# j-horner/cuda-nbody

Hardware: AMD Instinct MI355X
Metric: body-body interactions/s, all-pairs N-body step (reference convention N^2 per step) (higher is better)
Workload: dtype f32

## Files before the change

cuda-nbody_amd/csrc/nbody_pair.hip:

```cpp
#include "nbody_kernels.h"

#include <algorithm>
#include <cmath>
#include <vector>

#ifdef NB_PAIR_STAMPS
__device__ unsigned long long nb_pair_stamps[8192 * 8];
extern "C" __attribute__((visibility("default"))) int nb_debug_read_pair_stamps(void* host, size_t bytes) {
    return static_cast<int>(hipMemcpyFromSymbol(host, HIP_SYMBOL(nb_pair_stamps), bytes, 0, hipMemcpyDeviceToHost));
}
#endif

#ifdef NB_PAIR_NONTEMPORAL
#define NB_WS_STORE(ptr, value) __builtin_nontemporal_store((value), (ptr))
#define NB_WS_LOAD(ptr) __builtin_nontemporal_load(ptr)
#else
#define NB_WS_STORE(ptr, value) (*(ptr) = (value))
#define NB_WS_LOAD(ptr) (*(ptr))
#endif

namespace nb {
namespace {

#include "nbody_lane.h"

constexpr int kWaveRor1 = 0x13C;
__device__ __forceinline__ int rotate_bits(int v) { return __builtin_amdgcn_update_dpp(v, v, kWaveRor1, 0xf, 0xf, false); }
__device__ __forceinline__ float rotate(float x) { return __builtin_bit_cast(float, rotate_bits(__builtin_bit_cast(int, x))); }
__device__ __forceinline__ double rotate(double x) {
    const unsigned long long b  = __builtin_bit_cast(unsigned long long, x);
    const unsigned           l2 = static_cast<unsigned>(rotate_bits(static_cast<int>(b & 0xffffffffull)));
    const unsigned           h2 = static_cast<unsigned>(rotate_bits(static_cast<int>(b >> 32)));
    return __builtin_bit_cast(double, (static_cast<unsigned long long>(h2) << 32) | l2);
}
__device__ __forceinline__ v2f rotate(v2f x) { return v2f{rotate(x.x), rotate(x.y)}; }

__device__ __forceinline__ float first_lane(float x) { return __builtin_bit_cast(float, __builtin_amdgcn_readfirstlane(__builtin_bit_cast(int, x))); }
__device__ __forceinline__ double first_lane(double x) {
    const unsigned long long b  = __builtin_bit_cast(unsigned long long, x);
    const unsigned           lo = static_cast<unsigned>(__builtin_amdgcn_readfirstlane(static_cast<int>(b & 0xffffffffull)));
    const unsigned           hi = static_cast<unsigned>(__builtin_amdgcn_readfirstlane(static_cast<int>(b >> 32)));
    return __builtin_bit_cast(double, (static_cast<unsigned long long>(hi) << 32) | lo);
}

__device__ __forceinline__ float  both_halves(v2f a) { return a.x + a.y; }
__device__ __forceinline__ double both_halves(double a) { return a; }

template <int R, int S> constexpr int kPairWavesPerSimd = R <= 4 ? 4 : (S == 12 ? 3 : 2);
#define NB_PAIR_KERNEL pair_forces
#define NB_PAIR_CLOCK_PARAM
#define NB_PAIR_CLOCKED 0
#include "nbody_pair_forces.inc"
#undef NB_PAIR_KERNEL
#undef NB_PAIR_CLOCK_PARAM
#undef NB_PAIR_CLOCKED
#define NB_PAIR_KERNEL pair_forces_clocked
#define NB_PAIR_CLOCK_PARAM , unsigned long long* clock_words
#define NB_PAIR_CLOCKED 1
#include "nbody_pair_forces.inc"
#undef NB_PAIR_KERNEL
#undef NB_PAIR_CLOCK_PARAM
#undef NB_PAIR_CLOCKED

template <typename T> __device__ __forceinline__ void quarter_sums(const T* r, size_t plane, unsigned slots, unsigned wave, T (&t)[3]) {
    const unsigned full = slots & ~3u;
    t[0] = t[1] = t[2] = 0;
    for (unsigned q = wave; q < full; q += 32) {
        T v[3][8];
#pragma unroll
        for (int u = 0; u < 8; ++u) {
            const bool there = (q + 4 * u) < full;
#pragma unroll
            for (int c = 0; c < 3; ++c) v[c][u] = there ? NB_WS_LOAD(r + (static_cast<size_t>(q + 4 * u) * 3 + c) * plane) : T(0);
        }
#pragma unroll
        for (int u = 0; u < 8; ++u) {
#pragma unroll
            for (int c = 0; c < 3; ++c) t[c] += v[c][u];
        }
    }
    if (wave == 0) {
        for (unsigned k = full; k < slots; ++k) {
#pragma unroll
            for (int c = 0; c < 3; ++c) t[c] += NB_WS_LOAD(r + (static_cast<size_t>(k) * 3 + c) * plane);
        }
    }
}

template <typename T> __global__ __launch_bounds__(256) void pair_finish(FinishArgs<T> s) {
    using vec4 = typename Lane<T>::vec4;
    __shared__ T   part[3][3][64];
    const unsigned lane = threadIdx.x & 63, wave = threadIdx.x >> 6;
    const unsigned k    = blockIdx.x * 64 + lane;
    const bool     live = k < s.count;
    T              t[3] = {0, 0, 0};
    const unsigned body   = s.origin + k;
    const bool     closer = wave == 0 && live;
    vec4           v{}, pn{}, e{};
    T              own[3] = {0, 0, 0};
    if (closer) {
        v  = reinterpret_cast<const vec4*>(s.vel)[body];
        pn = reinterpret_cast<const vec4*>(s.old_pos)[body];
        if (s.extra != nullptr) e = reinterpret_cast<const vec4*>(s.extra)[body];
        for (unsigned m = 0; m < s.n_self; ++m) {
            const auto& set = s.self_set[m];
            if (k < set.first || k - set.first >= set.count) continue;
            for (unsigned c0 = 0; c0 < set.slots; c0 += 4) {
                T x[4][3];
#pragma unroll
                for (int i = 0; i < 4; ++i) {
#pragma unroll
                    for (int comp = 0; comp < 3; ++comp) x[i][comp] = (c0 + i) < set.slots ? NB_WS_LOAD(s.self + (static_cast<size_t>(set.slot + c0 + i) * 3 + comp) * s.self_plane + k) : T(0);
                }
#pragma unroll
                for (int i = 0; i < 4; ++i) {
                    if ((c0 + i) < set.slots) {
#pragma unroll
                        for (int comp = 0; comp < 3; ++comp) own[comp] += x[i][comp];
                    }
                }
            }
        }
    }
    if (live) quarter_sums(s.react + k, s.react_plane, s.react_slots, wave, t);
    if (wave != 0) {
#pragma unroll
        for (int comp = 0; comp < 3; ++comp) part[wave - 1][comp][lane] = t[comp];
    }
    __syncthreads();
    if (!closer) return;
    T    got[kMaxRecv][3];
    bool has[kMaxRecv];
#pragma unroll
    for (int m = 0; m < kMaxRecv; ++m) {
        has[m] = static_cast<unsigned>(m) < s.n_recv && k >= s.recv_set[m].first && k - s.recv_set[m].first < s.recv_set[m].count;
#pragma unroll
        for (int comp = 0; comp < 3; ++comp) got[m][comp] = has[m] ? s.recv[(static_cast<size_t>(m) * 3 + comp) * s.recv_plane + k] : T(0);
    }
    T f[3];
#pragma unroll
    for (int comp = 0; comp < 3; ++comp) {
        T others = (t[comp] + part[0][comp][lane]) + (part[1][comp][lane] + part[2][comp][lane]);
#pragma unroll
        for (int m = 0; m < kMaxRecv; ++m) {
            if (has[m]) others += got[m][comp];
        }
        f[comp] = own[comp] - others;
    }
    if (s.extra != nullptr) f[0] += e.x, f[1] += e.y, f[2] += e.z;
    v.x     = __builtin_fma(f[0], s.dt, v.x) * s.damping;
    v.y     = __builtin_fma(f[1], s.dt, v.y) * s.damping;
    v.z     = __builtin_fma(f[2], s.dt, v.z) * s.damping;
    pn.x    = __builtin_fma(v.x, s.dt, pn.x);
    pn.y    = __builtin_fma(v.y, s.dt, pn.y);
    pn.z    = __builtin_fma(v.z, s.dt, pn.z);
    reinterpret_cast<vec4*>(s.new_pos)[body] = pn;
    reinterpret_cast<vec4*>(s.vel)[body]     = v;
}

template <typename T> __global__ __launch_bounds__(256) void pair_reduce(const T* react, unsigned react_plane, unsigned slots, T* out, unsigned out_plane, unsigned count) {
    __shared__ T   part[3][3][64];
    const unsigned lane = threadIdx.x & 63, wave = threadIdx.x >> 6;
    const unsigned k    = blockIdx.x * 64 + lane;
    const bool     live = k < count;
    T              t[3] = {0, 0, 0};
    if (live) quarter_sums(react + k, react_plane, slots, wave, t);
    if (wave != 0) {
#pragma unroll
        for (int comp = 0; comp < 3; ++comp) part[wave - 1][comp][lane] = t[comp];
    }
    __syncthreads();
    if (wave != 0 || !live) return;
#pragma unroll
    for (int comp = 0; comp < 3; ++comp) out[static_cast<size_t>(comp) * out_plane + k] = (t[comp] + part[0][comp][lane]) + (part[1][comp][lane] + part[2][comp][lane]);
}

template <typename T, int R, int S> hipError_t launch_rs(const PairArgs<T>& args, unsigned grid, unsigned lds_bytes, hipStream_t stream, bool prepare_only) {
    if (lds_bytes > 64u * 1024u) {
        if (const auto err = allow_large_lds<&pair_forces<T, R, S>>(); err != hipSuccess) return err;
    }
    unsigned long long* clock_words = nullptr;
    if constexpr (R == 8 && S == 8) {
        size_t capacity = 0;
        unsigned long long* lent = pair_clock_words(&capacity);
        if (lent != nullptr && capacity >= static_cast<size_t>(grid) * 16) clock_words = lent;
        if (lds_bytes > 64u * 1024u && clock_words != nullptr) {
            if (const auto err = allow_large_lds<&pair_forces_clocked<T, R, S>>(); err != hipSuccess) return err;
        }
    }
    if (prepare_only) return hipSuccess;
    (void)hipGetLastError();
    if constexpr (R == 8 && S == 8) {
        if (clock_words != nullptr) {
            hipLaunchKernelGGL((pair_forces_clocked<T, R, S>), dim3(grid), dim3(64 * S), lds_bytes, stream, args, clock_words);
            return hipGetLastError();
        }
    }
    hipLaunchKernelGGL((pair_forces<T, R, S>), dim3(grid), dim3(64 * S), lds_bytes, stream, args);
    return hipGetLastError();
}

template <typename T, int R> hipError_t launch_r(const PairArgs<T>& args, int waves, unsigned grid, unsigned lds_bytes, hipStream_t stream, bool prepare_only) {
    switch (waves) {
        case 4: return launch_rs<T, R, 4>(args, grid, lds_bytes, stream, prepare_only);
        case 8: return launch_rs<T, R, 8>(args, grid, lds_bytes, stream, prepare_only);
        case 12: return launch_rs<T, R, 12>(args, grid, lds_bytes, stream, prepare_only);
        case 16: return launch_rs<T, R, 16>(args, grid, lds_bytes, stream, prepare_only);
        default: return hipErrorInvalidValue;
    }
}

}

inline double resident_workgroups(int S) { return 256.0 * std::max(1, 8 / S); }

inline double busiest_simd_units(unsigned U, unsigned C, int S, bool quarters) {
    const unsigned slots = C * static_cast<unsigned>(S), base = U / slots, rem = U % slots;
    const double   per_simd = static_cast<double>(S) / 4;
    if (quarters) return per_simd * base + pair_tail_units(U, C, S) / 4.0;
    const bool     inter = C > 1 && rem != 0 && base < 34;
    if (rem == 0) return per_simd * base;
    const unsigned longer = (inter || C == 1) ? (rem + C - 1) / C : std::min(rem, static_cast<unsigned>(S));
    return per_simd * base + (longer <= 4 ? 1.0 : 2.0);
}

template <typename T> struct PairCost;
template <> struct PairCost<float> {
    static constexpr double unit[4] = {2.2, 4.53, 9.17, 17.72}, wg[4] = {0.0, 0.0, 1.45, 6.86}, slot = 14.1;
};
template <> struct PairCost<double> {
    static constexpr double unit[4] = {0.0, 5.12, 10.39, 20.72}, wg[4] = {0.0, 0.0, 0.0, 0.0}, slot = 21.9;
};

template <typename T> PairPlan plan_pair(unsigned n, int cu_count, int ovr_r, int ovr_s, int ovr_c) {
    constexpr int W = sizeof(T) == 4 ? 2 : 1;
    (void)cu_count;
    const bool fixed_r = ovr_r == 1 || ovr_r == 2 || ovr_r == 4 || ovr_r == 8;
    const int  S       = (ovr_s == 4 || ovr_s == 8 || ovr_s == 12 || ovr_s == 16) ? ovr_s : 8;
    auto geometry = [&](int R, unsigned C) {
        PairPlan p{};
        const unsigned block  = 64u * static_cast<unsigned>(R * W);
        const unsigned blocks = (n + block - 1) / block;
        p.vectors_per_lane = R;
        p.waves            = S;
        p.splits           = C;
        p.blocks           = blocks;
        p.block_bodies     = block;
        p.slots            = blocks < 2 ? 0u : ((blocks & 1u) ? blocks / 2 : blocks / 2 - 1);
        p.grid_blocks      = blocks * C;
        p.lds_bytes        = pair_lds_bytes(R, W, S, sizeof(T), pair_tail_units((blocks / 2 + 1) * static_cast<unsigned>(R * W), C, S));
        if (p.lds_bytes > kPairLdsLimit) p.lds_bytes = pair_lds_bytes(R, W, S, sizeof(T), 0);
        p.workspace_bytes  = (static_cast<size_t>(C) + p.slots) * 3 * static_cast<size_t>(blocks) * block * sizeof(T);
        return p;
    };
    auto units_of = [&](const PairPlan& p) { return (p.blocks / 2 + 1) * static_cast<unsigned>(p.vectors_per_lane * W); };
    auto with_units = [&](int R, unsigned C) {
        PairPlan p = geometry(R, C);
        while (p.splits > 1 && units_of(p) < p.splits * static_cast<unsigned>(S)) p = geometry(R, p.splits / 2);
        return p;
    };
    PairPlan best{};
    double   best_cost = 0;
    for (int R : {1, 2, 4, 8}) {
        const int k = R == 1 ? 0 : (R == 2 ? 1 : (R == 4 ? 2 : 3));
        if (fixed_r ? R != ovr_r : PairCost<T>::unit[k] == 0.0) continue;
        for (unsigned C = 1; C <= 16; ++C) {
            const PairPlan p = ovr_c > 0 ? with_units(R, static_cast<unsigned>(ovr_c)) : geometry(R, C);
            const unsigned U = units_of(p);
            if (ovr_c <= 0 && C > 1 && U < 2 * C * static_cast<unsigned>(S)) continue;
            const double rounds = std::ceil(p.grid_blocks / resident_workgroups(S));
            const double unit   = PairCost<T>::unit[k] > 0.0 ? PairCost<T>::unit[k] : 0.5 * PairCost<T>::unit[1];
            const bool   quarters = pair_lds_bytes(R, W, S, sizeof(T), pair_tail_units(U, p.splits, S)) <= kPairLdsLimit;
            const double cost   = rounds * (busiest_simd_units(U, p.splits, S, quarters) * unit + PairCost<T>::wg[k]) +
                                PairCost<T>::slot * 1e-6 * static_cast<double>(n) * (p.slots + p.splits);
            if (best.blocks == 0 || cost < 0.995 * best_cost) best = p, best_cost = cost;
            if (ovr_c > 0) break;
        }
    }
    return best;
}

template <typename T> hipError_t launch_pair_tile(const PairArgs<T>& args, const PairGeom& g, hipStream_t stream, bool prepare_only) {
    constexpr int  W         = sizeof(T) == 4 ? 2 : 1;
    PairArgs<T>    a         = args;
    const unsigned block     = 64u * static_cast<unsigned>(g.vectors_per_lane * W);
    a.blocks                 = (a.i_count + block - 1) / block;
    a.splits                 = g.splits;
    const unsigned units = a.diag ? (a.unit_count != 0 ? a.unit_count : (a.blocks / 2 + 1) * static_cast<unsigned>(g.vectors_per_lane * W)) : (a.j_count + 63) / 64;
    unsigned       lds_bytes;
    {
        const unsigned slots = g.splits * static_cast<unsigned>(g.waves), each = units / slots;
        const unsigned tail  = pair_tail_units(units, g.splits, g.waves);
        lds_bytes            = pair_lds_bytes(g.vectors_per_lane, W, g.waves, sizeof(T), tail);
#ifdef NB_PAIR_NO_QUARTERS
        const bool quarters = false;
#else
        const bool quarters = lds_bytes <= kPairLdsLimit;
#endif
        if (quarters) {
            a.deal = 2u;
        } else {
            a.deal    = (g.splits > 1 && units % slots != 0 && each < 34) ? 1u : 0u;
            lds_bytes = pair_lds_bytes(g.vectors_per_lane, W, g.waves, sizeof(T), 0);
        }
    }
    if (a.blocks == 0) return hipSuccess;
    switch (g.vectors_per_lane) {
        case 1: return launch_r<T, 1>(a, g.waves, a.blocks * a.splits, lds_bytes, stream, prepare_only);
        case 2: return launch_r<T, 2>(a, g.waves, a.blocks * a.splits, lds_bytes, stream, prepare_only);
        case 4: return launch_r<T, 4>(a, g.waves, a.blocks * a.splits, lds_bytes, stream, prepare_only);
        case 8: return launch_r<T, 8>(a, g.waves, a.blocks * a.splits, lds_bytes, stream, prepare_only);
        default: return hipErrorInvalidValue;
    }
}

template <typename T> hipError_t launch_pair_reduce(const T* react, unsigned react_plane, unsigned slots, T* out, unsigned out_plane, unsigned count, hipStream_t stream) {
    if (count == 0) return hipSuccess;
    (void)hipGetLastError();
    hipLaunchKernelGGL(pair_reduce<T>, dim3((count + 63) / 64), dim3(256), 0, stream, react, react_plane, slots, out, out_plane, count);
    return hipGetLastError();
}

template <typename T> hipError_t launch_pair_finish(const FinishArgs<T>& args, hipStream_t stream) {
    if (args.count == 0) return hipSuccess;
    (void)hipGetLastError();
    hipLaunchKernelGGL(pair_finish<T>, dim3((args.count + 63) / 64), dim3(256), 0, stream, args);
    return hipGetLastError();
}

template <typename T> hipError_t launch_pair(const Shard<T>& s, const PairPlan& p, void* workspace, hipStream_t stream, bool prepare_only) {
    const unsigned npad = p.blocks * p.block_bodies;
    T* const       work = static_cast<T*>(workspace);
    PairArgs<T>    a{};
    a.old_pos = s.old_pos, a.self = work, a.react = work + static_cast<size_t>(p.splits) * 3 * npad;
    a.n = s.i_count, a.i_begin = 0, a.i_count = s.i_count, a.j_begin = 0, a.j_count = s.i_count;
    a.diag = 1, a.keep = 1;
    a.self_first = 0, a.self_origin = 0, a.self_plane = npad, a.react_origin = 0, a.react_plane = npad;
    a.eps2 = s.eps2;
    const PairGeom g{p.vectors_per_lane, p.waves, p.splits};
    if (const auto err = launch_pair_tile<T>(a, g, stream, prepare_only); err != hipSuccess || prepare_only) return err;
    if (hipEvent_t probe = pair_probe_event(); probe != nullptr) {
        if (const auto err = hipEventRecord(probe, stream); err != hipSuccess) return err;
    }
    FinishArgs<T> f{};
    f.old_pos = s.old_pos, f.new_pos = s.new_pos, f.vel = s.vel;
    f.self = a.self, f.react = a.react, f.recv = nullptr, f.extra = nullptr;
    f.origin = 0, f.count = s.i_count;
    f.self_plane = npad, f.react_plane = npad, f.react_slots = p.slots, f.recv_plane = 0;
    f.n_self = 1, f.n_recv = 0;
    f.self_set[0] = {0u, p.splits, 0u, s.i_count};
    f.dt = s.dt, f.damping = s.damping;
    return launch_pair_finish<T>(f, stream);
}

template <typename T> PairSlicing plan_pair_sliced(unsigned n, unsigned slices, int ovr_r, int ovr_s, int ovr_c) {
    constexpr unsigned W = sizeof(T) == 4 ? 2 : 1;
    PairSlicing        p{};
    if (n == 0 || slices < 2) return p;
    const int R = (ovr_r == 1 || ovr_r == 2 || ovr_r == 4 || ovr_r == 8) ? ovr_r : (n / slices >= 32768 ? 8 : 4);
    const int S = (ovr_s == 4 || ovr_s == 8 || ovr_s == 12 || ovr_s == 16) ? ovr_s : 8;
    const unsigned chip = 256u;
    p.block_bodies          = 64u * static_cast<unsigned>(R) * W;
    const unsigned blocks   = (n + p.block_bodies - 1) / p.block_bodies;
    const unsigned per      = (blocks + slices - 1) / slices;
    p.slice_bodies          = per * p.block_bodies;
    p.slices                = (n + p.slice_bodies - 1) / p.slice_bodies;
    if (p.slices < 2) return PairSlicing{};
    p.partners = p.slices / 2;
    p.even     = (p.slices % 2) == 0;
    if (p.partners + 1 > static_cast<unsigned>(kMaxRecv) || p.partners + 1 > static_cast<unsigned>(kMaxSelfSets)) return PairSlicing{};
    p.plane = p.slice_bodies;
    auto splits = [&](unsigned units) {
        unsigned C = ovr_c > 0 ? static_cast<unsigned>(ovr_c) : splits_to_fill(per, units, S, chip);
        while (C > 1 && units < C * static_cast<unsigned>(S)) C /= 2;
        return C;
    };
    p.diag = {R, S, splits((per / 2 + 1) * static_cast<unsigned>(R) * W)};
    p.rect = {R, S, splits(p.slice_bodies / 64)};
    p.rect_upper = p.rect;
    if (p.even && per >= 2 && p.slice_bodies / 64 >= p.rect.splits * 2 * static_cast<unsigned>(S) * 2) p.rect_upper.splits = p.rect.splits * 2;
    const size_t   plane3     = 3 * static_cast<size_t>(p.plane);
    const unsigned diag_slots = per < 2 ? 0u : ((per & 1u) ? per / 2 : per / 2 - 1);
    p.self_per_slice  = (p.diag.splits + static_cast<size_t>(p.partners - 1) * p.rect.splits + p.rect_upper.splits) * plane3;
    p.react_elements  = static_cast<size_t>(std::max(diag_slots, per)) * plane3;
    p.recv_per_slice  = (1 + static_cast<size_t>(p.partners)) * plane3;
    p.elements        = p.slices * (p.self_per_slice + p.recv_per_slice) + p.react_elements;
    p.workspace_bytes = p.elements * sizeof(T);
    return p;
}

template <typename T> hipError_t launch_pair_sliced(const Shard<T>& s, const PairSlicing& p, void* workspace, hipStream_t stream, bool prepare_only) {
    const unsigned n = s.i_count, K = p.slices, ni = p.slice_bodies, H = p.partners;
    const size_t   plane3 = 3 * static_cast<size_t>(p.plane);
    T* const       work   = static_cast<T*>(workspace);
    T* const       react  = work;
    auto self_of = [&](unsigned r) { return work + p.react_elements + static_cast<size_t>(r) * p.self_per_slice; };
    auto recv_of = [&](unsigned r) { return work + p.react_elements + static_cast<size_t>(K) * p.self_per_slice + static_cast<size_t>(r) * p.recv_per_slice; };
    auto first_of = [&](unsigned r) { return r * ni; };
    auto count_of = [&](unsigned r) { return std::min(ni, n - r * ni); };
    auto blocks_of = [&](unsigned count) { return (count + p.block_bodies - 1) / p.block_bodies; };
    auto half_of = [&](unsigned r) { return (blocks_of(count_of(r)) / 2) * p.block_bodies; };

    std::vector<FinishArgs<T>> finish(K);
    for (unsigned r = 0; r < K; ++r) {
        FinishArgs<T>& f = finish[r];
        f                = {};
        f.old_pos = s.old_pos, f.new_pos = s.new_pos, f.vel = s.vel;
        f.self = self_of(r), f.react = react, f.recv = recv_of(r), f.extra = nullptr;
        f.origin = first_of(r), f.count = count_of(r);
        f.self_plane = f.react_plane = f.recv_plane = p.plane;
        f.react_slots = 0;
        f.dt = s.dt, f.damping = s.damping;
        f.n_recv = 1 + H;
        for (unsigned m = 0; m <= H; ++m) f.recv_set[m] = {0u, 0u};
    }
    for (unsigned r = 0; r < K; ++r) {
        const unsigned own = first_of(r), cnt = count_of(r);
        PairArgs<T>    a{};
        a.old_pos = s.old_pos, a.self = self_of(r), a.n = n, a.eps2 = s.eps2;
        a.self_origin = own, a.self_plane = p.plane, a.react = react, a.react_plane = p.plane;
        a.react_origin = own, a.i_begin = a.j_begin = own, a.i_count = a.j_count = cnt, a.diag = 1, a.keep = 1, a.self_first = 0;
        if (const auto err = launch_pair_tile<T>(a, p.diag, stream, prepare_only); err != hipSuccess) return err;
        finish[r].self_set[finish[r].n_self++] = {0u, p.diag.splits, 0u, cnt};
        const unsigned b = blocks_of(cnt), diag_slots = b < 2 ? 0u : ((b & 1u) ? b / 2 : b / 2 - 1);
        if (diag_slots != 0) {
            if (!prepare_only) {
                if (const auto err = launch_pair_reduce<T>(react, p.plane, diag_slots, recv_of(r), p.plane, cnt, stream); err != hipSuccess) return err;
            }
            finish[r].recv_set[0] = {0u, cnt};
        }
        for (unsigned q = 1; q <= H; ++q) {
            const unsigned partner = (r + q) % K, pfirst = first_of(partner), pcnt = count_of(partner);
            a.diag = 0, a.keep = 1;
            a.i_begin = own, a.i_count = cnt, a.j_begin = pfirst, a.j_count = pcnt;
            const bool split = p.even && q == H;
            if (split) {
                if (r < partner) a.j_count = half_of(partner);
                else a.i_begin = own + half_of(r), a.i_count = cnt - half_of(r);
            }
            a.react_origin = a.j_begin;
            a.self_first   = p.diag.splits + (q - 1) * p.rect.splits;
            if (a.i_count != 0 && a.j_count != 0) {
                const PairGeom& geom = (split && !(r < partner)) ? p.rect_upper : p.rect;
                if (const auto err = launch_pair_tile<T>(a, geom, stream, prepare_only); err != hipSuccess) return err;
                finish[r].self_set[finish[r].n_self++] = {a.self_first, geom.splits, a.i_begin - own, a.i_count};
                if (!prepare_only) {
                    if (const auto err = launch_pair_reduce<T>(react, p.plane, blocks_of(a.i_count), recv_of(partner) + q * plane3, p.plane, a.j_count, stream); err != hipSuccess) return err;
                }
                finish[partner].recv_set[q] = {0u, a.j_count};
            }
        }
    }
    if (prepare_only) return hipSuccess;
    for (unsigned r = 0; r < K; ++r) {
        if (const auto err = launch_pair_finish<T>(finish[r], stream); err != hipSuccess) return err;
    }
    return hipSuccess;
}

template PairPlan   plan_pair<float>(unsigned, int, int, int, int);
template PairPlan   plan_pair<double>(unsigned, int, int, int, int);
template hipError_t launch_pair<float>(const Shard<float>&, const PairPlan&, void*, hipStream_t, bool);
template hipError_t launch_pair<double>(const Shard<double>&, const PairPlan&, void*, hipStream_t, bool);
template PairSlicing plan_pair_sliced<float>(unsigned, unsigned, int, int, int);
template PairSlicing plan_pair_sliced<double>(unsigned, unsigned, int, int, int);
template hipError_t  launch_pair_sliced<float>(const Shard<float>&, const PairSlicing&, void*, hipStream_t, bool);
template hipError_t  launch_pair_sliced<double>(const Shard<double>&, const PairSlicing&, void*, hipStream_t, bool);
template hipError_t launch_pair_tile<float>(const PairArgs<float>&, const PairGeom&, hipStream_t, bool);
template hipError_t launch_pair_tile<double>(const PairArgs<double>&, const PairGeom&, hipStream_t, bool);
template hipError_t launch_pair_reduce<float>(const float*, unsigned, unsigned, float*, unsigned, unsigned, hipStream_t);
template hipError_t launch_pair_reduce<double>(const double*, unsigned, unsigned, double*, unsigned, unsigned, hipStream_t);
template hipError_t launch_pair_finish<float>(const FinishArgs<float>&, hipStream_t);
template hipError_t launch_pair_finish<double>(const FinishArgs<double>&, hipStream_t);

}
```

Measured before the change: 7021 billion.

## Add specialized j-packed symmetric pair kernel for the 8-wave single-split config

Adds a new float-only pair-force kernel that packs two j bodies per lane as v2f. It rotates them across the wave with DPP, and accumulates reactions through a fused rotate-add DPP. Wave priority is adjusted from per-SIMD progress counters, and the kernel is dispatched in place of the generic tile kernel when the plan is 8 vectors per lane, 8 waves and one split. The intent is to raise throughput in the inner loop through more ILP and fewer j loads. The risks are higher register pressure, a separate code path to keep consistent with the generic kernel, and LDS sizing that reuses the generic formula.

```diff
diff --git a/cuda-nbody_amd/csrc/nbody_pair.hip b/cuda-nbody_amd/csrc/nbody_pair.hip
--- a/cuda-nbody_amd/csrc/nbody_pair.hip
+++ b/cuda-nbody_amd/csrc/nbody_pair.hip
@@ -1,8 +1,15 @@
 #include "nbody_kernels.h"
+#include "nbody_pair_lead.h"
 
 #include <algorithm>
 #include <cmath>
 #include <vector>
+
+#if defined(NB_PAIR_STAMPS) || defined(NB_PAIR_NONTEMPORAL) || defined(NB_NO_BALANCE) || defined(NB_PAIR_NO_QUARTERS) || defined(NB_PAIR_UNR) || defined(NB_PAIR_RB)
+#define NB_PAIR_VARIANT_BUILD 1
+#else
+#define NB_PAIR_VARIANT_BUILD 0
+#endif
 
 #ifdef NB_PAIR_STAMPS
 __device__ unsigned long long nb_pair_stamps[8192 * 8];
@@ -11,40 +18,11 @@
 }
 #endif
 
-#ifdef NB_PAIR_NONTEMPORAL
-#define NB_WS_STORE(ptr, value) __builtin_nontemporal_store((value), (ptr))
-#define NB_WS_LOAD(ptr) __builtin_nontemporal_load(ptr)
-#else
-#define NB_WS_STORE(ptr, value) (*(ptr) = (value))
-#define NB_WS_LOAD(ptr) (*(ptr))
-#endif
-
 namespace nb {
 namespace {
 
 #include "nbody_lane.h"
-
-constexpr int kWaveRor1 = 0x13C;
-__device__ __forceinline__ int rotate_bits(int v) { return __builtin_amdgcn_update_dpp(v, v, kWaveRor1, 0xf, 0xf, false); }
-__device__ __forceinline__ float rotate(float x) { return __builtin_bit_cast(float, rotate_bits(__builtin_bit_cast(int, x))); }
-__device__ __forceinline__ double rotate(double x) {
-    const unsigned long long b  = __builtin_bit_cast(unsigned long long, x);
-    const unsigned           l2 = static_cast<unsigned>(rotate_bits(static_cast<int>(b & 0xffffffffull)));
-    const unsigned           h2 = static_cast<unsigned>(rotate_bits(static_cast<int>(b >> 32)));
-    return __builtin_bit_cast(double, (static_cast<unsigned long long>(h2) << 32) | l2);
-}
-__device__ __forceinline__ v2f rotate(v2f x) { return v2f{rotate(x.x), rotate(x.y)}; }
-
-__device__ __forceinline__ float first_lane(float x) { return __builtin_bit_cast(float, __builtin_amdgcn_readfirstlane(__builtin_bit_cast(int, x))); }
-__device__ __forceinline__ double first_lane(double x) {
-    const unsigned long long b  = __builtin_bit_cast(unsigned long long, x);
-    const unsigned           lo = static_cast<unsigned>(__builtin_amdgcn_readfirstlane(static_cast<int>(b & 0xffffffffull)));
-    const unsigned           hi = static_cast<unsigned>(__builtin_amdgcn_readfirstlane(static_cast<int>(b >> 32)));
-    return __builtin_bit_cast(double, (static_cast<unsigned long long>(hi) << 32) | lo);
-}
-
-__device__ __forceinline__ float  both_halves(v2f a) { return a.x + a.y; }
-__device__ __forceinline__ double both_halves(double a) { return a; }
+#include "nbody_pair_lane.h"
 
 template <int R, int S> constexpr int kPairWavesPerSimd = R <= 4 ? 4 : (S == 12 ? 3 : 2);
 #define NB_PAIR_KERNEL pair_forces
@@ -338,7 +316,14 @@
     a.self_first = 0, a.self_origin = 0, a.self_plane = npad, a.react_origin = 0, a.react_plane = npad;
     a.eps2 = s.eps2;
     const PairGeom g{p.vectors_per_lane, p.waves, p.splits};
-    if (const auto err = launch_pair_tile<T>(a, g, stream, prepare_only); err != hipSuccess || prepare_only) return err;
+    const bool lead = !NB_PAIR_VARIANT_BUILD && pair_lead_takes(a, g);
+    if (lead) {
+        if (const auto err = launch_pair_lead(a, stream, prepare_only); err != hipSuccess) return err;
+    }
+    if (!lead || prepare_only) {
+        if (const auto err = launch_pair_tile<T>(a, g, stream, prepare_only); err != hipSuccess) return err;
+    }
+    if (prepare_only) return hipSuccess;
     if (hipEvent_t probe = pair_probe_event(); probe != nullptr) {
         if (const auto err = hipEventRecord(probe, stream); err != hipSuccess) return err;
     }
diff --git a/cuda-nbody_amd/csrc/nbody_pair_lane.h b/cuda-nbody_amd/csrc/nbody_pair_lane.h
--- /dev/null
+++ b/cuda-nbody_amd/csrc/nbody_pair_lane.h
@@ -0,0 +1,34 @@
+#pragma once
+
+#ifdef NB_PAIR_NONTEMPORAL
+#define NB_WS_STORE(ptr, value) __builtin_nontemporal_store((value), (ptr))
+#define NB_WS_LOAD(ptr) __builtin_nontemporal_load(ptr)
+#else
+#define NB_WS_STORE(ptr, value) (*(ptr) = (value))
+#define NB_WS_LOAD(ptr) (*(ptr))
+#endif
+
+constexpr int kWaveRor1 = 0x13C;
+__device__ __forceinline__ int rotate_bits(int v) { return __builtin_amdgcn_update_dpp(v, v, kWaveRor1, 0xf, 0xf, false); }
+__device__ __forceinline__ float rotate(float x) { return __builtin_bit_cast(float, rotate_bits(__builtin_bit_cast(int, x))); }
+__device__ __forceinline__ double rotate(double x) {
+    const unsigned long long b  = __builtin_bit_cast(unsigned long long, x);
+    const unsigned           l2 = static_cast<unsigned>(rotate_bits(static_cast<int>(b & 0xffffffffull)));
+    const unsigned           h2 = static_cast<unsigned>(rotate_bits(static_cast<int>(b >> 32)));
+    return __builtin_bit_cast(double, (static_cast<unsigned long long>(h2) << 32) | l2);
+}
+__device__ __forceinline__ v2f rotate(v2f x) { return v2f{rotate(x.x), rotate(x.y)}; }
+__device__ __forceinline__ float rotate_add(float x, float t) {
+    return __builtin_bit_cast(float, __builtin_amdgcn_update_dpp(0, __builtin_bit_cast(int, x), kWaveRor1, 0xf, 0xf, true)) + t;
+}
+
+__device__ __forceinline__ float first_lane(float x) { return __builtin_bit_cast(float, __builtin_amdgcn_readfirstlane(__builtin_bit_cast(int, x))); }
+__device__ __forceinline__ double first_lane(double x) {
+    const unsigned long long b  = __builtin_bit_cast(unsigned long long, x);
+    const unsigned           lo = static_cast<unsigned>(__builtin_amdgcn_readfirstlane(static_cast<int>(b & 0xffffffffull)));
+    const unsigned           hi = static_cast<unsigned>(__builtin_amdgcn_readfirstlane(static_cast<int>(b >> 32)));
+    return __builtin_bit_cast(double, (static_cast<unsigned long long>(hi) << 32) | lo);
+}
+
+__device__ __forceinline__ float  both_halves(v2f a) { return a.x + a.y; }
+__device__ __forceinline__ double both_halves(double a) { return a; }
diff --git a/cuda-nbody_amd/csrc/nbody_pair_lead.h b/cuda-nbody_amd/csrc/nbody_pair_lead.h
--- /dev/null
+++ b/cuda-nbody_amd/csrc/nbody_pair_lead.h
@@ -0,0 +1,13 @@
+#pragma once
+
+#include "nbody_kernels.h"
+
+namespace nb {
+
+bool       pair_lead_takes(const PairArgs<float>& args, const PairGeom& g);
+inline bool pair_lead_takes(const PairArgs<double>&, const PairGeom&) { return false; }
+
+hipError_t       launch_pair_lead(const PairArgs<float>& args, hipStream_t stream, bool prepare_only);
+inline hipError_t launch_pair_lead(const PairArgs<double>&, hipStream_t, bool) { return hipErrorInvalidValue; }
+
+}
diff --git a/cuda-nbody_amd/csrc/nbody_pair_lead.hip b/cuda-nbody_amd/csrc/nbody_pair_lead.hip
--- /dev/null
+++ b/cuda-nbody_amd/csrc/nbody_pair_lead.hip
@@ -0,0 +1,299 @@
+#include "nbody_pair_lead.h"
+
+namespace nb {
+namespace {
+
+#include "nbody_lane.h"
+#include "nbody_pair_lane.h"
+
+#ifndef NB_PAIR_LEAD_UNR
+#define NB_PAIR_LEAD_UNR 1
+#endif
+#ifndef NB_PAIR_LEAD_IB
+#define NB_PAIR_LEAD_IB 4
+#endif
+
+template <int S> __global__ __launch_bounds__(64 * S) __attribute__((amdgpu_waves_per_eu(2, 2))) void pair_forces_jpacked(PairArgs<float> s) {
+    using LT            = Lane<float>;
+    using T             = float;
+    using vec           = v2f;
+    constexpr int I     = 16;
+    constexpr int P     = I / 2;
+    constexpr int BLOCK = 64 * I;
+    constexpr int TB    = I / 2;
+    constexpr int UNR   = NB_PAIR_LEAD_UNR;
+
+    extern __shared__ __attribute__((aligned(32))) unsigned char smem_raw[];
+
+    const float4* __restrict__ old_pos = reinterpret_cast<const float4*>(s.old_pos);
+    const int      tid  = threadIdx.x;
+    const int      wave = __builtin_amdgcn_readfirstlane(tid >> 6);
+    const int      lane = tid & 63;
+    const unsigned a    = blockIdx.x;
+
+    const unsigned block_base = s.i_begin + a * BLOCK;
+    const unsigned i_end      = s.i_begin + s.i_count;
+    vec            px[P], py[P], pz[P];
+    vec            ax[I], ay[I], az[I];
+    const T        m_block    = old_pos[block_base < i_end ? block_base : i_end - 1].w;
+    const unsigned block_bits = __builtin_bit_cast(unsigned, m_block);
+    bool           same       = true;
+#pragma unroll
+    for (int k = 0; k < I; ++k) {
+        const unsigned i = block_base + k * 64 + lane;
+        const float4   p = old_pos[i < i_end ? i : i_end - 1];
+        LT::set(px[k / 2], k % 2, p.x);
+        LT::set(py[k / 2], k % 2, p.y);
+        LT::set(pz[k / 2], k % 2, p.z);
+        same = same && i < i_end && __builtin_bit_cast(unsigned, p.w) == block_bits;
+    }
+    const bool block_uniform = __builtin_amdgcn_ballot_w64(!same) == 0 && usable_scale(m_block);
+#pragma unroll
+    for (int k = 0; k < I; ++k) ax[k] = ay[k] = az[k] = LT::splat(0);
+    vec eps2 = LT::splat(s.eps2);
+    LT::keep_in_vgpr(eps2);
+    const LT::Consts consts = LT::make_consts();
+
+    constexpr size_t kSumBytes = static_cast<size_t>(S) * 3 * I * 64 * sizeof(T);
+    T* const         sums      = reinterpret_cast<T*>(smem_raw);
+    unsigned* const  balance   = reinterpret_cast<unsigned*>(smem_raw + kSumBytes);
+    unsigned* const  simd_count = balance;
+    volatile unsigned* progress = reinterpret_cast<volatile unsigned*>(balance + 4);
+    if (tid < 36) balance[tid] = tid < 4 ? 0u : 0xffffffffu;
+    __syncthreads();
+    const unsigned simd = static_cast<unsigned>(__builtin_amdgcn_s_getreg((1 << 11) | (4 << 6) | 4));
+    unsigned       slot = 0;
+    if (lane == 0) slot = atomicAdd(&simd_count[simd], 1u);
+    slot = static_cast<unsigned>(__builtin_amdgcn_readfirstlane(static_cast<int>(slot))) & 7u;
+    volatile unsigned* const mine = progress + simd * 8;
+    unsigned                 done = 0;
+    if (lane == 0) mine[slot] = 0;
+
+    constexpr unsigned kFlush = 8;
+    T* const           second = sums + static_cast<size_t>(wave) * (3 * I * 64) + lane;
+#pragma unroll
+    for (int q = 0; q < 3 * I; ++q) second[q * 64] = 0;
+    T unit = T(1);
+    auto flush = [&](vec (&ax)[I], vec (&ay)[I], vec (&az)[I]) {
+#pragma unroll
+        for (int k = 0; k < I; ++k) {
+            second[(0 * I + k) * 64] = __builtin_fmaf(both_halves(ax[k]), unit, second[(0 * I + k) * 64]);
+            second[(1 * I + k) * 64] = __builtin_fmaf(both_halves(ay[k]), unit, second[(1 * I + k) * 64]);
+            second[(2 * I + k) * 64] = __builtin_fmaf(both_halves(az[k]), unit, second[(2 * I + k) * 64]);
+        }
+#pragma unroll
+        for (int k = 0; k < I; ++k) ax[k] = ay[k] = az[k] = LT::splat(0);
+    };
+    auto change_unit = [&](T to) {
+        const vec ratio = LT::splat(unit / to);
+#pragma unroll
+        for (int k = 0; k < I; ++k) ax[k] = ax[k] * ratio, ay[k] = ay[k] * ratio, az[k] = az[k] * ratio;
+        unit = to;
+    };
+
+    const unsigned NB      = s.blocks;
+    const unsigned Q       = NB / 2;
+    const bool     even    = (NB & 1u) == 0;
+    const unsigned j_end   = s.j_begin + s.j_count;
+    const unsigned n_units = (Q + 1) * TB;
+    const unsigned n_items = static_cast<unsigned>(wave) < n_units ? (n_units - static_cast<unsigned>(wave) + S - 1) / S : 0;
+    auto item_unit = [&](unsigned it) { return static_cast<unsigned>(wave) + it * S; };
+    auto tile_first = [&](unsigned u) {
+        unsigned jb = a + u / TB;
+        if (jb >= NB) jb -= NB;
+        return s.j_begin + jb * BLOCK + (u % TB) * 128;
+    };
+    struct Tile {
+        float4 lo, hi;
+    };
+    auto load_tile = [&](unsigned u) {
+        const unsigned j = tile_first(u) + static_cast<unsigned>(lane);
+        return Tile{old_pos[j < j_end ? j : j_end - 1], old_pos[j + 64 < j_end ? j + 64 : j_end - 1]};
+    };
+
+    struct Reaction {
+        float x0, x1, y0, y1, z0, z1;
+    };
+    auto step = [&]<bool MASSES>(vec (&ax)[I], vec (&ay)[I], vec (&az)[I], vec (&px)[P], vec (&py)[P], vec (&pz)[P], vec& jx, vec& jy, vec& jz, vec& jm, Reaction& re, vec (&mi)[P]) {
+        constexpr int IB = NB_PAIR_LEAD_IB;
+#pragma unroll
+        for (int p = 0; p < P; ++p) {
+            LT::keep_in_vgpr(px[p]), LT::keep_in_vgpr(py[p]), LT::keep_in_vgpr(pz[p]);
+            if constexpr (MASSES) LT::keep_in_vgpr(mi[p]);
+        }
+        vec tx, ty, tz;
+#pragma unroll
+        for (int h = 0; h < I; h += IB) {
+            vec dx[IB], dy[IB], dz[IB], w[IB];
+#pragma unroll
+            for (int r = 0; r < IB; ++r) {
+                const int k = h + r;
+                dx[r] = jx - LT::splat(LT::get(px[k / 2], k % 2)), dy[r] = jy - LT::splat(LT::get(py[k / 2], k % 2)), dz[r] = jz - LT::splat(LT::get(pz[k / 2], k % 2));
+            }
+#pragma unroll
+            for (int r = 0; r < IB; ++r) w[r] = LT::fma(dx[r], dx[r], eps2);
+#pragma unroll
+            for (int r = 0; r < IB; ++r) w[r] = LT::fma(dy[r], dy[r], w[r]);
+#pragma unroll
+            for (int r = 0; r < IB; ++r) w[r] = LT::fma(dz[r], dz[r], w[r]);
+#pragma unroll
+            for (int r = 0; r < IB; ++r) w[r] = LT::coupling_rel<true>(eps2, w[r], consts);
+#pragma unroll
+            for (int r = 0; r < IB; ++r) {
+                const int k  = h + r;
+                vec       wi = w[r], wj = w[r];
+                if constexpr (MASSES) wi = jm * w[r], wj = LT::splat(LT::get(mi[k / 2], k % 2)) * w[r];
+                ax[k] = LT::fma(dx[r], wi, ax[k]), ay[k] = LT::fma(dy[r], wi, ay[k]), az[k] = LT::fma(dz[r], wi, az[k]);
+                if (k == 0) tx = dx[r] * wj, ty = dy[r] * wj, tz = dz[r] * wj;
+                else tx = LT::fma(dx[r], wj, tx), ty = LT::fma(dy[r], wj, ty), tz = LT::fma(dz[r], wj, tz);
+            }
+        }
+        jx = rotate(jx), jy = rotate(jy), jz = rotate(jz);
+        if constexpr (MASSES) jm = rotate(jm);
+        re.x0 = rotate_add(re.x0, tx.x), re.x1 = rotate_add(re.x1, tx.y);
+        re.y0 = rotate_add(re.y0, ty.x), re.y1 = rotate_add(re.y1, ty.y);
+        re.z0 = rotate_add(re.z0, tz.x), re.z1 = rotate_add(re.z1, tz.y);
+    };
+    auto rotation_steps = [&]<bool MASSES>(vec (&ax)[I], vec (&ay)[I], vec (&az)[I], vec (&px)[P], vec (&py)[P], vec (&pz)[P], vec& jx, vec& jy, vec& jz, vec& jm, Reaction& re, vec (&mi)[P]) {
+#pragma unroll 1
+        for (int it = 0; it < 64 / UNR; ++it) {
+#pragma unroll
+            for (int v = 0; v < UNR; ++v) step.template operator()<MASSES>(ax, ay, az, px, py, pz, jx, jy, jz, jm, re, mi);
+        }
+    };
+
+    Tile cur = n_items > 0 ? load_tile(item_unit(0)) : Tile{};
+    for (unsigned item = 0; item < n_items; ++item) {
+        const unsigned u    = item_unit(item);
+        const Tile     next = (item + 1) < n_items ? load_tile(item_unit(item + 1)) : cur;
+        {
+            unsigned least = done;
+#pragma unroll
+            for (int q = 0; q < 8; ++q) least = min(least, mine[q]);
+            if (static_cast<unsigned>(__builtin_amdgcn_readfirstlane(static_cast<int>(least))) >= done) {
+                __builtin_amdgcn_s_setprio(3);
+            } else {
+                __builtin_amdgcn_s_setprio(0);
+            }
+        }
+        const unsigned q     = u / TB;
+        const unsigned j     = tile_first(u) + static_cast<unsigned>(lane);
+        if (j >= j_end) cur.lo.w = 0;
+        if (j + 64 >= j_end) cur.hi.w = 0;
+        const T    m_tile      = first_lane(cur.lo.w);
+        const bool one_species = block_uniform && usable_unit(m_tile) &&
+                                 __builtin_amdgcn_ballot_w64(!(j + 64 < j_end && __builtin_bit_cast(unsigned, cur.lo.w) == __builtin_bit_cast(unsigned, m_tile) &&
+                                                               __builtin_bit_cast(unsigned, cur.hi.w) == __builtin_bit_cast(unsigned, m_tile))) == 0;
+        vec jx = vec{cur.lo.x, cur.hi.x}, jy = vec{cur.lo.y, cur.hi.y}, jz = vec{cur.lo.z, cur.hi.z}, jm = LT::splat(0);
+        Reaction re{};
+        T   scale = T(1);
+        if (one_species) {
+            if (__builtin_bit_cast(unsigned, m_tile) != __builtin_bit_cast(unsigned, unit)) change_unit(m_tile);
+            scale = m_block;
+            vec none[P] = {};
+            rotation_steps.template operator()<false>(ax, ay, az, px, py, pz, jx, jy, jz, jm, re, none);
+        } else {
+            jm = vec{cur.lo.w, cur.hi.w} / LT::splat(unit);
+            vec mi[P];
+#pragma unroll
+            for (int k = 0; k < I; ++k) {
+                const unsigned i = block_base + k * 64 + lane;
+                LT::set(mi[k / 2], k % 2, i < i_end ? old_pos[i].w : T(0));
+            }
+            vec gx[P], gy[P], gz[P];
+#pragma unroll
+            for (int p = 0; p < P; ++p) gx[p] = px[p], gy[p] = py[p], gz[p] = pz[p];
+            flush(ax, ay, az);
+            vec bx[I], by[I], bz[I];
+#pragma unroll
+            for (int k = 0; k < I; ++k) bx[k] = by[k] = bz[k] = LT::splat(0);
+            rotation_steps.template operator()<true>(bx, by, bz, gx, gy, gz, jx, jy, jz, jm, re, mi);
+            flush(bx, by, bz);
+        }
+        re.x0 = rotate(re.x0), re.x1 = rotate(re.x1), re.y0 = rotate(re.y0), re.y1 = rotate(re.y1), re.z0 = rotate(re.z0), re.z1 = rotate(re.z1);
+        const bool symmetric = q != 0 && !(even && q == Q);
+        if (symmetric) {
+            T* const out = s.react + static_cast<size_t>(q - 1) * 3 * s.react_plane + (j - s.react_origin);
+            if (j < j_end) {
+                NB_WS_STORE(out, re.x0 * scale);
+                NB_WS_STORE(out + static_cast<size_t>(s.react_plane), re.y0 * scale);
+                NB_WS_STORE(out + 2 * static_cast<size_t>(s.react_plane), re.z0 * scale);
+            }
+            if (j + 64 < j_end) {
+                NB_WS_STORE(out + 64, re.x1 * scale);
+                NB_WS_STORE(out + static_cast<size_t>(s.react_plane) + 64, re.y1 * scale);
+                NB_WS_STORE(out + 2 * static_cast<size_t>(s.react_plane) + 64, re.z1 * scale);
+            }
+        }
+        cur = next;
+        ++done;
+        if (done % kFlush == 0) flush(ax, ay, az);
+        if (lane == 0) mine[slot] = done;
+    }
+    if (lane == 0) mine[slot] = 0xffffffffu;
+    __builtin_amdgcn_s_setprio(0);
+
+    T fx[I], fy[I], fz[I];
+#pragma unroll
+    for (int k = 0; k < I; ++k) {
+        fx[k] = second[(0 * I + k) * 64] + both_halves(ax[k]) * unit;
+        fy[k] = second[(1 * I + k) * 64] + both_halves(ay[k]) * unit;
+        fz[k] = second[(2 * I + k) * 64] + both_halves(az[k]) * unit;
+    }
+
+    __syncthreads();
+    T* const red = sums;
+    if (wave > 0) {
+#pragma unroll
+        for (int k = 0; k < I; ++k) {
+            red[(((wave - 1) * 3 + 0) * I + k) * 64 + lane] = fx[k];
+            red[(((wave - 1) * 3 + 1) * I + k) * 64 + lane] = fy[k];
+            red[(((wave - 1) * 3 + 2) * I + k) * 64 + lane] = fz[k];
+        }
+    }
+    __syncthreads();
+    if (wave != 0) return;
+#pragma unroll 1
+    for (int w = 1; w < S; ++w) {
+#pragma unroll
+        for (int k = 0; k < I; ++k) {
+            fx[k] += red[(((w - 1) * 3 + 0) * I + k) * 64 + lane];
+            fy[k] += red[(((w - 1) * 3 + 1) * I + k) * 64 + lane];
+            fz[k] += red[(((w - 1) * 3 + 2) * I + k) * 64 + lane];
+        }
+    }
+    T* const self = s.self + static_cast<size_t>(s.self_first) * 3 * s.self_plane;
+#pragma unroll
+    for (int k = 0; k < I; ++k) {
+        const unsigned i = block_base + k * 64 + lane;
+        if (i >= i_end) continue;
+        const size_t at = i - s.self_origin;
+        NB_WS_STORE(self + at, fx[k]);
+        NB_WS_STORE(self + static_cast<size_t>(s.self_plane) + at, fy[k]);
+        NB_WS_STORE(self + 2 * static_cast<size_t>(s.self_plane) + at, fz[k]);
+    }
+}
+
+}
+
+bool pair_lead_takes(const PairArgs<float>& a, const PairGeom& g) {
+    size_t bytes = 0;
+    return g.vectors_per_lane == 8 && g.waves == 8 && g.splits == 1 && a.diag != 0 && a.unit_begin == 0 && a.unit_count == 0 && a.i_count != 0 &&
+           pair_clock_words(&bytes) == nullptr &&
+           pair_probe_event() == nullptr;
+}
+
+hipError_t launch_pair_lead(const PairArgs<float>& args, hipStream_t stream, bool prepare_only) {
+    constexpr int  S     = 8;
+    PairArgs<float> a    = args;
+    a.blocks             = (a.i_count + 1023u) / 1024u;
+    a.splits             = 1;
+    const unsigned lds_bytes = pair_lds_bytes(8, 2, S, sizeof(float), 0);
+    if (const auto err = allow_large_lds<&pair_forces_jpacked<S>>(); err != hipSuccess) return err;
+    if (prepare_only) return hipSuccess;
+    (void)hipGetLastError();
+    hipLaunchKernelGGL((pair_forces_jpacked<S>), dim3(a.blocks), dim3(64 * S), lds_bytes, stream, a);
+    return hipGetLastError();
+}
+
+}
```

Measured after the change: 7170 billion (median of 6 runs). 2.1% higher.
